# funcwj/setk

Measured on AMD Instinct MI355X. Metric: real-time-factor (audio-sec/wall-sec), 8-ch 16 kHz MVDR, higher is better.
Workload: dtype f32; 1 GPU; 8-ch 16 kHz oracle-mask MVDR, 30 s utterances, 125 per GPU (BASELINE configs[2] shard: 1000 at 8 GPUs), STFT 512/256/hann/center, inputs resident in HBM; utts_per_gpu=125, channels=8, frames=1876, beamformer=mvdr, parallelism=utterance-sharded x1

## Files before the change

setk_amd/build.py:

```python
import os
import subprocess
import sys
from concurrent.futures import ThreadPoolExecutor

HERE = os.path.dirname(os.path.abspath(__file__))
CSRC = os.path.join(HERE, "csrc")
OBJ = os.path.join(CSRC, "_obj")
LIB = os.path.join(HERE, "libsetk_hip.so")
SOURCES = ["pass1.hip", "pass1_mc.hip", "pass2.hip", "pass2_mc.hip", "solve.hip", "modular.hip", "cgmm.hip", "cgmm_bin.hip", "cgmm_k.hip", "wpe.hip", "auxiva.hip", "comm.hip", "hostio.hip",
           "capi_support.hip", "capi_handle.hip", "capi_stft.hip", "capi_modular.hip", "capi_fused.hip", "capi_cgmm.hip", "capi_wpe.hip", "capi_auxiva.hip"]
HEADERS = ["common.h", "fft512.h", "dpp.h", "covar_fold.h", "mcdft.h", "mcdft_tables.h", "capi.h", os.path.join("..", "..", "include", "setk_hip.h")]
ARCH = "gfx950"


def _hipcc():
    for cand in (os.environ.get("HIPCC"), "/opt/rocm/bin/hipcc", "hipcc"):
        if cand and (os.path.isabs(cand) and os.path.exists(cand) or not os.path.isabs(cand)):
            return cand
    return "hipcc"


def _stale(target, deps):
    if not os.path.exists(target):
        return True
    t = os.path.getmtime(target)
    return any(os.path.getmtime(d) > t for d in deps)


def build_library(force=False, verbose=False):
    os.makedirs(OBJ, exist_ok=True)
    import fcntl
    with open(os.path.join(OBJ, ".lock"), "w") as lock:
        fcntl.flock(lock, fcntl.LOCK_EX)
        return _build_locked(force, verbose)


def _build_locked(force, verbose):
    hdrs = [os.path.normpath(os.path.join(CSRC, h)) for h in HEADERS]
    flags = ["--offload-arch=" + ARCH, "-O3", "-std=c++17", "-fPIC", "-ffp-contract=fast",
             "-fno-slp-vectorize",
             "-Wno-unused-result"] + os.environ.get("SETK_HIPCC_FLAGS", "").split()
    extra = {"pass1.hip": ["-mllvm", "-amdgpu-sched-strategy=max-memory-clause"],
             "pass2_mc.hip": ["-mllvm", "-amdgpu-sched-strategy=max-ilp"],
             "pass2.hip": ["-mllvm", "-amdgpu-sched-strategy=max-ilp"],
             "solve.hip": ["-mllvm", "-amdgpu-sched-strategy=max-ilp"],
             "modular.hip": ["-mllvm", "-amdgpu-sched-strategy=max-ilp"],
             "cgmm.hip": ["-mllvm", "-amdgpu-sched-strategy=max-ilp"],
             "cgmm_bin.hip": ["-mllvm", "-amdgpu-sched-strategy=iterative-ilp"],
             "cgmm_k.hip": [],
             "wpe.hip": ["-mllvm", "-amdgpu-sched-strategy=max-ilp"],
             "auxiva.hip": [],
             "comm.hip": []}
    honor = {"solve.hip", "modular.hip"}
    jobs = []
    objs = []
    for src in SOURCES:
        s = os.path.join(CSRC, src)
        o = os.path.join(OBJ, src.replace(".hip", ".o"))
        objs.append(o)
        if force or _stale(o, [s] + hdrs):
            fl = [f if f != "-ffp-contract=fast" or src not in honor else "-ffp-contract=fast-honor-pragmas"
                  for f in flags]
            jobs.append([_hipcc()] + fl + extra.get(src, []) + ["-c", s, "-o", o])

    def run(cmd):
        if verbose:
            print(" ".join(cmd), file=sys.stderr)
        r = subprocess.run(cmd, capture_output=True, text=True)
        if r.returncode != 0:
            raise RuntimeError("hipcc failed:\n" + " ".join(cmd) + "\n" + r.stdout + r.stderr)
        return r

    if jobs:
        with ThreadPoolExecutor(max_workers=min(len(jobs), os.cpu_count() or 1)) as ex:
            list(ex.map(run, jobs))
    if force or jobs or _stale(LIB, objs):
        run([_hipcc(), "--offload-arch=" + ARCH, "-shared", "-fPIC", "-o", LIB] + objs)
    return LIB


if __name__ == "__main__":
    if "--units" in sys.argv:
        print(" ".join(s[:-len(".hip")] for s in SOURCES))
        sys.exit(0)
    print(build_library(force="--force" in sys.argv, verbose=True))
```

setk_amd/csrc/fft512.h:

```cpp
#pragma once
#include <hip/hip_runtime.h>

namespace setk {

typedef float2 cf;

#define SETK_DEV __device__ __forceinline__

#define SETK_GLOBAL __attribute__((address_space(1)))
typedef const SETK_GLOBAL float* gcfloat_p;
typedef float v2f __attribute__((ext_vector_type(2)));
typedef const SETK_GLOBAL v2f* gcfloat2_p;
template <class T>
SETK_DEV const SETK_GLOBAL T* gptr(const T* p) {
    return (const SETK_GLOBAL T*)p;
}

SETK_DEV cf cadd(cf a, cf b) { return make_float2(a.x + b.x, a.y + b.y); }
SETK_DEV cf csub(cf a, cf b) { return make_float2(a.x - b.x, a.y - b.y); }
SETK_DEV cf cmul(cf a, cf b) {
    return make_float2(a.x * b.x - a.y * b.y, a.x * b.y + a.y * b.x);
}
SETK_DEV cf cmulc(cf a, cf b) {
    return make_float2(a.x * b.x + a.y * b.y, a.y * b.x - a.x * b.y);
// ... 35 lines not shown
    v[4 * 1 + 1] = twid16<DIR, 1>(v[4 * 1 + 1]);
    v[4 * 2 + 1] = twid16<DIR, 2>(v[4 * 2 + 1]);
    v[4 * 3 + 1] = twid16<DIR, 3>(v[4 * 3 + 1]);
    v[4 * 1 + 2] = twid16<DIR, 2>(v[4 * 1 + 2]);
    v[4 * 2 + 2] = twid16<DIR, 4>(v[4 * 2 + 2]);
    v[4 * 3 + 2] = twid16<DIR, 6>(v[4 * 3 + 2]);
    v[4 * 1 + 3] = twid16<DIR, 3>(v[4 * 1 + 3]);
    v[4 * 2 + 3] = twid16<DIR, 6>(v[4 * 2 + 3]);
    v[4 * 3 + 3] = twid16<DIR, 9>(v[4 * 3 + 3]);
#pragma unroll
    for (int c = 0; c < 4; ++c)
        dft4<DIR>(v[4 * c], v[4 * c + 1], v[4 * c + 2], v[4 * c + 3]);
}

constexpr int kRow5 = 10;
__host__ __device__ constexpr int slot_entries(int row) { return 16 * row; }
__host__ __device__ constexpr int table_entries(int row) {
    return (row % 2 == 0) ? 2 * 16 * row + 16 * kRow5 : 640;
}
template <int ROW> struct LaneTab {
    static constexpr bool rows = (ROW % 2 == 0);
    static constexpr int estride = rows ? 1 : 16;
    static constexpr int lstride = rows ? ROW : 1;
    static constexpr int lstride5 = rows ? kRow5 : 1;
    static constexpr int size = rows ? 16 * ROW : 256;
};

template <int N, bool WIDE = true>
SETK_DEV void lds_row(const cf* row, cf (&out)[N]) {
    if (WIDE) {
        const float4* r4 = reinterpret_cast<const float4*>(__builtin_assume_aligned(row, 16));
#pragma unroll
        for (int n = 0; n < N / 2; ++n) {
            const float4 t = r4[n];
            out[2 * n] = make_float2(t.x, t.y);
            out[2 * n + 1] = make_float2(t.z, t.w);
        }
    } else {
#pragma unroll
        for (int n = 0; n < N; ++n) out[n] = row[n];
    }
}

template <int ROW>
SETK_DEV void fill_lane_tables(cf* win_l, cf* tw_l, cf* tw5_l, const float* window,
                               const float2* tw256, const float2* tw512, int tid, int nthreads) {
    for (int i = tid; i < 256; i += nthreads) {
        const int la = i & 15, j = i >> 4, n = la + 16 * j;
        typedef LaneTab<ROW> L;
        win_l[la * L::lstride + j * L::estride] = make_float2(window[2 * n], window[2 * n + 1]);
        tw_l[la * L::lstride + j * L::estride] = tw256[j * 16 + la];
    }
    for (int i = tid; i < 128; i += nthreads) {
        const int la = i & 15, m = i >> 4;
        tw5_l[la * LaneTab<ROW>::lstride5 + m * LaneTab<ROW>::estride] = tw512[la + 16 * m];
    }
}

template <int ROW>
SETK_DEV void apply_window(cf (&v)[16], const cf* win_row) {
    if (LaneTab<ROW>::rows) {
        const float4* w4 = reinterpret_cast<const float4*>(__builtin_assume_aligned(win_row, 16));
#pragma unroll
        for (int j = 0; j < 16; j += 2) {
            const float4 w = w4[j / 2];
            v[j] = make_float2(v[j].x * w.x, v[j].y * w.y);
            v[j + 1] = make_float2(v[j + 1].x * w.z, v[j + 1].y * w.w);
        }
    } else {
#pragma unroll
        for (int j = 0; j < 16; ++j) {
            const cf w = win_row[j * 16];
            v[j] = make_float2(v[j].x * w.x, v[j].y * w.y);
        }
    }
}

template <int DIR, int ROW, bool WIDE = (ROW % 2 == 0)>
SETK_DEV void fft256_stage_a_pad(cf (&v)[16], cf* slot, const cf* tw_row, int la) {
    dft16<DIR>(v);
    cf* dst = slot + la;
    if (WIDE) {
        const float4* w4 = reinterpret_cast<const float4*>(__builtin_assume_aligned(tw_row, 16));
#pragma unroll
        for (int q = 0; q < 16; q += 2) {
            const float4 w = w4[q / 2];
            cf t0 = v[dft16_pos(q)], t1 = v[dft16_pos(q + 1)];
            if (q) t0 = cmul(t0, make_float2(w.x, DIR > 0 ? -w.y : w.y));
            t1 = cmul(t1, make_float2(w.z, DIR > 0 ? -w.w : w.w));
            dst[q * ROW] = t0;
            dst[(q + 1) * ROW] = t1;
        }
    } else {
        cf wq[16];
        wq[1] = tw_row[16];
        wq[2] = tw_row[32];
#pragma unroll
        for (int q = 0; q < 16; ++q) {
            if (q + 3 < 16) wq[q + 3] = tw_row[(q + 3) * 16];
            cf t = v[dft16_pos(q)];
            if (q) {
                cf w = wq[q];
                if (DIR > 0) w.y = -w.y;
                t = cmul(t, w);
            }
            dst[q * ROW] = t;
        }
    }
}

template <int DIR, int ROW, bool WIDE = (ROW % 2 == 0)>
SETK_DEV void fft256_stage_b_pad(cf (&v)[16], const cf* slot, int la) {
    lds_row<16, WIDE>(slot + la * ROW, v);
    dft16<DIR>(v);
}

SETK_DEV void rfft_split(cf Zk, cf Zm, cf w, cf& Xk, cf& Xm) {
    cf A = make_float2(Zk.x + Zm.x, Zk.y - Zm.y);
    cf O = make_float2(Zk.y + Zm.y, Zm.x - Zk.x);
    cf B = cmul(w, O);
    Xk = cadd(A, B);
    Xm = make_float2(A.x - B.x, -(A.y - B.y));
}

SETK_DEV void irfft_merge(cf Yk, cf Ym, cf w, cf& Zk, cf& Zm) {
    cf E = make_float2(Yk.x + Ym.x, Yk.y - Ym.y);
    cf D = make_float2(Yk.x - Ym.x, Yk.y + Ym.y);
    cf O = cmulc(D, w);
    Zk = make_float2(E.x - O.y, E.y + O.x);
    Zm = make_float2(E.x + O.y, -E.y + O.x);
}

constexpr int kFrame = 512;

SETK_DEV int reflect_index(int i, int n) {
    if (i < 0) i = -i;
    if (i >= n) i = 2 * (n - 1) - i;
    return i;
}

template <class FloatPtr> struct RawPair;
template <> struct RawPair<gcfloat_p> {
    typedef gcfloat2_p ptr;
    static SETK_DEV cf get(ptr p, int i) {
        const v2f d = p[i];
        return make_float2(d.x, d.y);
    }
};
template <> struct RawPair<const float*> {
    typedef const float2* ptr;
    static SETK_DEV cf get(ptr p, int i) { return p[i]; }
};

template <class FloatPtr>
SETK_DEV void load_raw(cf (&v)[16], FloatPtr x, int n_samp, int s, int la, bool valid) {
    if (!valid) {
#pragma unroll
        for (int j = 0; j < 16; ++j) v[j] = make_float2(0.f, 0.f);
        return;
    }
    const bool interior = (s >= 0) && (s + kFrame <= n_samp) && ((((uintptr_t)(x + s)) & 7) == 0);
    if (interior) {
        typename RawPair<FloatPtr>::ptr p = (typename RawPair<FloatPtr>::ptr)(x + s);
#pragma unroll
        for (int j = 0; j < 16; ++j) v[j] = RawPair<FloatPtr>::get(p, la + 16 * j);
    } else {
#pragma unroll
        for (int j = 0; j < 16; ++j) {
            const int n = la + 16 * j;
            v[j] = make_float2(x[reflect_index(s + 2 * n, n_samp)],
                               x[reflect_index(s + 2 * n + 1, n_samp)]);
        }
    }
}

typedef const SETK_GLOBAL short* gcshort_p;
typedef const SETK_GLOBAL int* gcint_p;
SETK_DEV void load_raw_pcm(int (&v)[16], gcshort_p x, int n_samp, int s, int la, bool valid) {
    if (!valid) {
#pragma unroll
        for (int j = 0; j < 16; ++j) v[j] = 0;
        return;
    }
    const bool interior = (s >= 0) && (s + kFrame <= n_samp) && ((((uintptr_t)(x + s)) & 3) == 0);
    if (interior) {
        gcint_p p = (gcint_p)(x + s);
#pragma unroll
        for (int j = 0; j < 16; ++j) v[j] = p[la + 16 * j];
    } else {
#pragma unroll
        for (int j = 0; j < 16; ++j) {
            const int n = la + 16 * j;
            const int lo = x[reflect_index(s + 2 * n, n_samp)];
            const int hi = x[reflect_index(s + 2 * n + 1, n_samp)];
            v[j] = (lo & 0xffff) | (hi << 16);
        }
    }
}
SETK_DEV cf unpack_pcm(int v) { return make_float2((float)(short)(v & 0xffff), (float)(v >> 16)); }

SETK_DEV float qr_partner(float x) {
    int v = __builtin_bit_cast(int, x);
    v = __builtin_amdgcn_update_dpp(0, v, 0x140, 0xf, 0xf, true);
    v = __builtin_amdgcn_update_dpp(0, v, 0x121, 0xf, 0xf, true);
    return __builtin_bit_cast(float, v);
}

template <int ROW, bool WIDE = (ROW % 2 == 0)>
SETK_DEV void qr_stage23(cf* slot, float* nyq, const cf* tw5_row, int la) {
    cf v[16];
    fft256_stage_b_pad<-1, ROW, WIDE>(v, slot, la);
    const bool lane0 = (la == 0);
    cf* lo = slot + la;
    cf* mir = slot + (256 - 16 * 7) - la;
    cf t5[8];
    if (WIDE) {
        lds_row<8, true>(tw5_row, t5);
    } else {
        t5[0] = tw5_row[0];
        t5[1] = tw5_row[16];
    }
#pragma unroll
    for (int m = 0; m < 8; ++m) {
        if (!WIDE && m + 2 < 8) t5[m + 2] = tw5_row[16 * (m + 2)];
        const cf Zk = v[dft16_pos(m)];
        const cf src = v[dft16_pos(15 - m)];
        cf Zm = make_float2(qr_partner(src.x), qr_partner(src.y));
        const cf own = v[dft16_pos((16 - m) & 15)];
        Zm.x = lane0 ? own.x : Zm.x;
        Zm.y = lane0 ? own.y : Zm.y;
        cf Xk, Xm;
        rfft_split(Zk, Zm, t5[m], Xk, Xm);
        if (m == 0) {
            const cf Z128 = v[dft16_pos(8)];
            if (lane0) {
                slot[0] = make_float2(Xk.x, 0.f);
                *nyq = Xm.x;
                slot[128] = make_float2(2.f * Z128.x, -2.f * Z128.y);
            } else {
                lo[16 * m] = Xk;
                mir[16 * (7 - m)] = Xm;
            }
        } else {
            lo[16 * m] = Xk;
            mir[16 * (7 - m)] = Xm;
        }
    }
}

}
```

setk_amd/csrc/pass1.hip:

```cpp
#include "common.h"
#include "fft512.h"
#include "covar_fold.h"
#include <cstdio>
#include <type_traits>
#include <cstdlib>

namespace setk {

template <int C, bool DUMP, bool PCM = false>
__global__ __launch_bounds__(1024, 4) void stft_covar_kernel(Pass1Args a) {
    constexpr int NT = 1024;
    constexpr int TB = pass1_tile_frames(C);
    constexpr int NF = TB * C;
    constexpr int NP = npairs(C);
    constexpr int ND = PairSplit<C>::ND, NO = PairSplit<C>::NO;
    constexpr int NS = 32 / NF;
    constexpr int F = kBins, FP = kBinsPad;
    constexpr int ROW = 17;
    constexpr int SL = slot_entries(ROW);

    extern __shared__ __attribute__((aligned(16))) char smem[];
    cf* xt0 = reinterpret_cast<cf*>(smem);
    cf* win_l = xt0 + 2 * NF * SL;
    cf* tw_l = win_l + LaneTab<ROW>::size;
// ... 110 lines not shown
                for (int j = i; j < C; ++j) {
                    if (cnt == e) { ny_i = i; ny_j = j; }
                    ++cnt;
                }
        }
        float cur_s[TB], cur_n[TB], nxt_s[TB], nxt_n[TB];
        auto fetch_masks = [&](int tb_tile, float (&ms)[TB], float (&mn)[TB]) {
#pragma unroll
            for (int tt = 0; tt < TB; ++tt) {
                const int t = tb_tile + tt;
                float vs = 0.f, vn = 0.f;
                if (t < wi.t1) {
                    vs = gptr(ud.mask_s)[(size_t)t * F + f];
                    if (has_mn) vn = gptr(ud.mask_n)[(size_t)t * F + f];
                }
                ms[tt] = vs;
                mn[tt] = vn;
            }
        };
        if (!DUMP) fetch_masks(wi.t0, cur_s, cur_n);
        wg_barrier();
        wg_barrier();
        int buf = 0;
#pragma unroll 1
        for (int tb = wi.t0; tb < wi.t1; tb += TB, buf ^= 1) {
            const cf* xt = xt0 + buf * NF * SL;
            const float* xn = xn0 + buf * 32;
            if (DUMP) {
                for (int i = q; i < NF; i += 2) {
                    const int tt = i / C, c = i - tt * C;
                    const int t = tb + tt;
                    if (t < wi.t1) {
                        float2* base = a.spec_dump ? reinterpret_cast<float2*>(a.spec_dump)
                                                   : reinterpret_cast<float2*>(ud.wave_out);
                        float2* dst = base + ((size_t)c * T + t) * (a.dump_pitch ? a.dump_pitch : F);
                        dst[f] = xt[i * SL + f];
                        if (f == 0) dst[256] = make_float2(xn[i], 0.f);
                    }
                }
            } else {
                if (tb + TB < wi.t1) fetch_masks(tb + TB, nxt_s, nxt_n);
#pragma unroll
                for (int tt = 0; tt < TB; ++tt) {
                    cf x[C];
#pragma unroll
                    for (int c = 0; c < C; ++c) x[c] = xt[(tt * C + c) * SL + f];
                    const bool fvalid = tb + tt < wi.t1;
                    const float ws = clamp ? fminf(cur_s[tt], 1.f) : cur_s[tt];
                    const float wn = fvalid ? (has_mn ? cur_n[tt] : 1.f - ws) : 0.f;
                    if (q == 0) {
                        aux0 += ws;
                        aux1 += wn;
                        accumulate_half<C, 0>(x, ws, wn, dg_s, dg_n, of_s, of_n);
                    } else {
                        accumulate_half<C, 1>(x, ws, wn, dg_s, dg_n, of_s, of_n);
                    }
                    if (ny_active) {
                        const float prod_ny =
                            (ny_item < 2 * NP) ? xn[tt * C + ny_i] * xn[tt * C + ny_j] : 1.f;
                        const bool speech = (ny_item < NP) || (ny_item == 2 * NP);
                        const float w256 = nym[(buf * 2 + (speech ? 0 : 1)) * 8 + tt];
                        aux0 = fmaf(w256, prod_ny, aux0);
                    }
                }
#pragma unroll
                for (int tt = 0; tt < TB; ++tt) {
                    cur_s[tt] = nxt_s[tt];
                    cur_n[tt] = nxt_n[tt];
                }
            }
            wg_barrier();
        }
    }

    if (!DUMP) {
        if (wi.last) {
            const int covered = (T - 1) * a.g.hop - a.g.pad + kNfft;
            for (int c = 0; c < C; ++c)
                for (int i = covered + tid; i < n_samp; i += NT) {
                    if constexpr (PCM)
                        mx = fmaxf(mx, fabsf((float)((gcshort_p)gptr(ud.audio))[(size_t)c * ud.ch_stride + i]));
                    else
                        mx = fmaxf(mx, fabsf(gptr(ud.audio)[(size_t)c * n_samp + i]));
                }
        }
        if constexpr (PCM) mx *= 3.0517578125e-05f;
#pragma unroll
        for (int o = 32; o > 0; o >>= 1) mx = fmaxf(mx, __shfl_xor(mx, o));
        if ((tid & 63) == 0) red[tid >> 6] = mx;
        __syncthreads();
        if (tid == 0) {
            float bm = red[0];
#pragma unroll
            for (int w = 1; w < NT / 64; ++w) bm = fmaxf(bm, red[w]);
            atomicMax(a.norm_bits + wi.utt, __float_as_uint(bm));
        }
        if (wave >= 8) {
            float* P = a.partials + (size_t)wi.part * nplanes_partial(C) * FP;
            if (q == 0) {
                store_half<C, 0>(P, f, dg_s, dg_n, of_s, of_n);
                P[(4 * NP + 0) * FP + f] = aux0;
                P[(4 * NP + 1) * FP + f] = aux1;
            } else {
                store_half<C, 1>(P, f, dg_s, dg_n, of_s, of_n);
            }
            if (ny_active) {
                if (ny_item < NP) {
                    P[(0 * NP + ny_item) * FP + 256] = aux0;
                    P[(1 * NP + ny_item) * FP + 256] = 0.f;
                } else if (ny_item < 2 * NP) {
                    P[(2 * NP + ny_item - NP) * FP + 256] = aux0;
                    P[(3 * NP + ny_item - NP) * FP + 256] = 0.f;
                } else {
                    P[(4 * NP + ny_item - 2 * NP) * FP + 256] = aux0;
                }
            }
        }
    }
}

constexpr int kBmFrames = 64;
constexpr int kBmSlot = slot_entries(17) + 1;

__global__ __launch_bounds__(1024, 4) void stft_binmajor_kernel(Pass1Args a, int C) {
    constexpr int ROW = 17;
    constexpr int NT = 1024;
    extern __shared__ __attribute__((aligned(16))) char smem[];
    cf* xt = reinterpret_cast<cf*>(smem);
    cf* win_l = xt + kBmFrames * kBmSlot;
    cf* tw_l = win_l + LaneTab<ROW>::size;
    cf* tw5_l = tw_l + LaneTab<ROW>::size;
    float* xn = reinterpret_cast<float*>(win_l + table_entries(ROW));

    const int tid = threadIdx.x;
    const int wave = tid >> 6, lane = tid & 63;
    const int la = tid & 15, grp = tid >> 4;
    const WorkItem wi = a.items[blockIdx.x];
    const UttDesc ud = a.utts[wi.utt];
    const int n_samp = ud.num_samples, T = ud.num_frames;
    const int Tp = (T + 3) & ~3;
    cf* out = reinterpret_cast<cf*>(ud.wave_out);
    fill_lane_tables<ROW>(win_l, tw_l, tw5_l, a.window, a.tw256, a.tw512, tid, NT);
    const cf* win_row = win_l + la * LaneTab<ROW>::lstride;
    const cf* tw_row = tw_l + la * LaneTab<ROW>::lstride;
    const cf* tw5_row = tw5_l + la * LaneTab<ROW>::lstride5;
    cf* slot = xt + grp * kBmSlot;
    const int t = wi.t0 + grp;
    const bool valid = t < wi.t1;

    const int s0 = t * a.g.hop - a.g.pad;
    __syncthreads();
    for (int c = 0; c < C; ++c) {
        cf v[16];
        load_raw(v, gptr(ud.audio) + (size_t)c * n_samp, n_samp, s0, la, valid);
        apply_window<ROW>(v, win_row);
        fft256_stage_a_pad<-1, ROW>(v, slot, tw_row, la);
        __builtin_amdgcn_wave_barrier();
        qr_stage23<ROW>(slot, xn + grp, tw5_row, la);
        __syncthreads();
        {
            const int fr = 2 * (lane & 31), half = lane >> 5;
            const int t2 = wi.t0 + fr;
            for (int f = 2 * wave + half; f < kBins; f += 2 * (NT / 64)) {
                cf v0, v1;
                if (f < 256) {
                    v0 = xt[fr * kBmSlot + f];
                    v1 = xt[(fr + 1) * kBmSlot + f];
                } else {
                    v0 = make_float2(xn[fr], 0.f);
                    v1 = make_float2(xn[fr + 1], 0.f);
                }
                cf* dst = out + ((size_t)f * C + c) * Tp + t2;
                if (t2 + 1 < wi.t1)
                    *reinterpret_cast<float4*>(dst) = make_float4(v0.x, v0.y, v1.x, v1.y);
                else if (t2 < wi.t1)
                    *dst = v0;
            }
        }
        __syncthreads();
    }
}

hipError_t launch_stft_binmajor(int C, const Pass1Args& a, int n_items, hipStream_t s) {
    const size_t lds = (size_t)kBmFrames * kBmSlot * sizeof(cf) + table_entries(17) * sizeof(cf) +
                       kBmFrames * sizeof(float);
    hipError_t e = hipFuncSetAttribute(reinterpret_cast<const void*>(stft_binmajor_kernel),
                                       hipFuncAttributeMaxDynamicSharedMemorySize, (int)lds);
    if (e != hipSuccess) return e;
    hipLaunchKernelGGL(stft_binmajor_kernel, dim3(n_items), dim3(1024), lds, s, a, C);
    return hipGetLastError();
}

template <int C, bool DUMP, bool PCM = false>
static hipError_t launch_pass1_t(const Pass1Args& a, int n_items, hipStream_t s) {
    constexpr int NF = pass1_tile_frames(C) * C;
    const size_t lds = (size_t)2 * NF * slot_entries(17) * sizeof(cf) + table_entries(17) * sizeof(cf) +
                       (64 + 32 + 16) * sizeof(float);
    auto k = stft_covar_kernel<C, DUMP, PCM>;
    hipError_t e = hipFuncSetAttribute(reinterpret_cast<const void*>(k),
                                       hipFuncAttributeMaxDynamicSharedMemorySize, (int)lds);
    if (e != hipSuccess) return e;
    hipLaunchKernelGGL(k, dim3(n_items), dim3(1024), lds, s, a);
    return hipGetLastError();
}

hipError_t launch_pass1(int C, bool dump, const Pass1Args& a, int n_items, hipStream_t s, bool pcm16) {
    if (pcm16 && dump) return hipErrorInvalidValue;
#define SETK_CASE(c)                                                \
    case c:                                                         \
        if (dump) return launch_pass1_t<c, true>(a, n_items, s);     \
        if (pcm16) return launch_pass1_t<c, false, true>(a, n_items, s); \
        return launch_pass1_t<c, false>(a, n_items, s);
    switch (C) {
        SETK_CASE(1)
        SETK_CASE(2)
        SETK_CASE(3)
        SETK_CASE(4)
        SETK_CASE(5)
        SETK_CASE(6)
        SETK_CASE(7)
        SETK_CASE(8)
    }
#undef SETK_CASE
    return hipErrorInvalidValue;
}

__global__ __launch_bounds__(320) void covar_finalize_kernel(FinalizeArgs a) {
    const int f = threadIdx.x;
    const int u = blockIdx.z;
    const int C = a.num_channels;
    const int NP = npairs(C);
    const int planes_in = 4 * NP + 2;
    const int planes_out = a.with_ry ? 6 * NP : 4 * NP;
    const int e = blockIdx.y;
    if (f >= kBinsPad) return;
    const UttDesc ud = a.utts[u];
    float* out = a.covar + ((size_t)u * planes_out + e) * kBinsPad;
    if (f >= kBins) {
        out[f] = 0.f;
        return;
    }
    const float* P = a.partials + (size_t)ud.part0 * planes_in * kBinsPad;
    const size_t slab = (size_t)planes_in * kBinsPad;
    if (e < 4 * NP) {
        const int sel = e / (2 * NP);
        float acc = 0.f, den = 0.f;
        for (int p = 0; p < ud.nparts; ++p) {
            acc += P[p * slab + (size_t)e * kBinsPad + f];
            den += P[p * slab + (size_t)(4 * NP + sel) * kBinsPad + f];
        }
        const float sc = a.num_scale / fmaxf(den, 1e-6f);
        out[f] = acc * sc;
    } else {
        const int r = e - 4 * NP;
        float acc = 0.f;
        for (int p = 0; p < ud.nparts; ++p)
            acc += P[p * slab + (size_t)r * kBinsPad + f] +
                   P[p * slab + (size_t)(2 * NP + r) * kBinsPad + f];
        const float sc = a.num_scale / fmaxf((float)ud.num_frames, 1e-6f);
        out[f] = acc * sc;
    }
}

hipError_t launch_finalize(const FinalizeArgs& a, int n_utts, hipStream_t s) {
    const int NP = npairs(a.num_channels);
    const int planes_out = a.with_ry ? 6 * NP : 4 * NP;
    dim3 grid(1, planes_out, n_utts);
    hipLaunchKernelGGL(covar_finalize_kernel, grid, dim3(320), 0, s, a);
    return hipGetLastError();
}

}
```

setk_amd/csrc/pass2_mc.hip:

```cpp
#include "common.h"
#include "fft512.h"
#include "mcdft.h"
#include <cstdio>
#include <cstdlib>
#include <type_traits>

namespace setk {

constexpr int kP2McWavesPerSimd = 4;
constexpr int kP2McGroup = 2;
constexpr int p2mc_threads(bool pcm) { return pcm ? 1024 : 512; }

constexpr int kP2McTiles = 25;
size_t pass2_mc_lds_bytes(int C, bool pcm) {
    const size_t nw = p2mc_threads(pcm) / 64;
    const size_t wt = ((size_t)C * kBins * sizeof(cf) + 15) & ~(size_t)15;
    return wt + kP2McTiles * 1024 + 2048 + nw * kP2McGroup * 8 * mc::kOddPitch * sizeof(float) +
           nw * kP2McGroup * 16 * sizeof(float) + 64 + (pcm ? nw * C * 64 * sizeof(uint2) : 0);
}

SETK_DEV float row8_sum(float x) {
    int v = __builtin_bit_cast(int, x);
    x += __builtin_bit_cast(float, __builtin_amdgcn_update_dpp(0, v, 0xB1, 0xf, 0xf, true));
    v = __builtin_bit_cast(int, x);
    x += __builtin_bit_cast(float, __builtin_amdgcn_update_dpp(0, v, 0x4E, 0xf, 0xf, true));
    v = __builtin_bit_cast(int, x);
    x += __builtin_bit_cast(float, __builtin_amdgcn_update_dpp(0, v, 0x141, 0xf, 0xf, true));
    return x;
}
SETK_DEV float wave_max_nonneg(float x) {
    int v = __builtin_bit_cast(int, x);
    x = fmaxf(x, __builtin_bit_cast(float, __builtin_amdgcn_update_dpp(0, v, 0xB1, 0xf, 0xf, true)));
    v = __builtin_bit_cast(int, x);
    x = fmaxf(x, __builtin_bit_cast(float, __builtin_amdgcn_update_dpp(0, v, 0x4E, 0xf, 0xf, true)));
    v = __builtin_bit_cast(int, x);
    x = fmaxf(x, __builtin_bit_cast(float, __builtin_amdgcn_update_dpp(0, v, 0x141, 0xf, 0xf, true)));
    v = __builtin_bit_cast(int, x);
    x = fmaxf(x, __builtin_bit_cast(float, __builtin_amdgcn_update_dpp(0, v, 0x140, 0xf, 0xf, true)));
    const unsigned b = __builtin_bit_cast(unsigned, x);
    unsigned m = __builtin_amdgcn_readlane(b, 0);
    const unsigned m1 = __builtin_amdgcn_readlane(b, 16), m2 = __builtin_amdgcn_readlane(b, 32),
                   m3 = __builtin_amdgcn_readlane(b, 48);
    m = m > m1 ? m : m1;
    m = m > m2 ? m : m2;
    m = m > m3 ? m : m3;
    return __builtin_bit_cast(float, m);
}

template <int C, bool PCM = false>
__global__ __launch_bounds__(p2mc_threads(PCM), kP2McWavesPerSimd) void beamform_istft_mc_kernel(Pass2Args a) {
    constexpr int NT = p2mc_threads(PCM);
    constexpr int NW = NT / 64;
    constexpr int F = kBins;

    extern __shared__ __attribute__((aligned(16))) char smem[];
    char* p = smem;
    cf* wtab = reinterpret_cast<cf*>(p);
    p += ((size_t)C * F * sizeof(cf) + 15) & ~(size_t)15;
    mc::u4* tiles = reinterpret_cast<mc::u4*>(p);
    p += kP2McTiles * 1024;
    mc::f4* synr = reinterpret_cast<mc::f4*>(p);
    p += 2048;
    float* a16s = reinterpret_cast<float*>(p);
    p += (size_t)NW * kP2McGroup * 8 * mc::kOddPitch * sizeof(float);
    float* yodd_s = reinterpret_cast<float*>(p);
    p += NW * kP2McGroup * 16 * sizeof(float);
    float* red = reinterpret_cast<float*>(p);
    p += 64;
    uint2* carry_s = reinterpret_cast<uint2*>(p);

    const int tid = threadIdx.x;
    const int lane = tid & 63;
    const int wave = __builtin_amdgcn_readfirstlane(tid >> 6);
    const int c16 = lane & 15, g = lane >> 4;
    const WorkItem wi = a.items[blockIdx.x];
    const UttDesc ud = a.utts[wi.utt];
    const int n_samp = ud.num_samples;
    const int T = ud.num_frames;
    const int hop = kNfft / 2;
    const bool post_mask = (a.flags & 0x4) != 0;
    const bool clamp = (a.flags & 0x2) != 0;

    float in_sc = PCM ? 3.0517578125e-05f : 1.f, out_sc = 1.f;
    if (a.norm_bits) {
        const unsigned nb = a.norm_bits[wi.utt];
        int e = (int)((nb >> 23) & 0xff) - 126;
        e = (__builtin_bit_cast(float, nb) <= 1.f) ? 0 : (e > 100 ? 100 : e);
        in_sc *= __builtin_bit_cast(float, (unsigned)(127 - e) << 23);
        out_sc = __builtin_bit_cast(float, (unsigned)(127 + e) << 23);
    }
    {
        const cf* wsrc = reinterpret_cast<const cf*>(a.weight) + (size_t)wi.utt * C * kBinsPad;
        for (int i = tid; i < C * F; i += NT) {
            const int c = i / F, f = i - c * F;
            wtab[i] = wsrc[c * kBinsPad + f];
        }
    }
    mc::stage_tiles(tiles, a.mc_tab, mc::kW_BR_H, 10, tid, NT);
    mc::stage_tiles(tiles + 10 * 64, a.mc_tab, mc::kW_OT_H, 2, tid, NT);
    mc::stage_tiles(tiles + 12 * 64, a.mc_tab, mc::kW_MC_H, 8, tid, NT);
    for (int i = tid; i < 128; i += NT) {
        const int l = i & 63, t4 = i >> 6;
        const mc::f4 w = {a.mc_win[(4 * t4 + 0) * 64 + l] * in_sc, a.mc_win[(4 * t4 + 1) * 64 + l] * in_sc,
                          a.mc_win[(4 * t4 + 2) * 64 + l] * in_sc, a.mc_win[(4 * t4 + 3) * 64 + l] * in_sc};
        tiles[20 * 64 + i] = __builtin_bit_cast(mc::u4, w);
    }
    mc::stage_tiles(tiles + 22 * 64, a.mc_tab, mc::kW_TR, 3, tid, NT);
    for (int i = tid; i < 128; i += NT) {
        const int l = i & 63, hf = i >> 6;
        synr[i] = (mc::f4){a.mc_syn[(4 * hf + 0) * 64 + l] * out_sc, a.mc_syn[(4 * hf + 1) * 64 + l] * out_sc,
                           a.mc_syn[(4 * hf + 2) * 64 + l] * out_sc, a.mc_syn[(4 * hf + 3) * 64 + l] * out_sc};
    }
    struct { float tr[4], ti[4]; } K;
    float* yoddw = yodd_s + wave * kP2McGroup * 16;
    const int lane_bin = mc::bin_of(c16, g, 0);
    const cf* wl = wtab + lane_bin;
    const int lane_n = 64 * g + c16;
    float omax = 0.f;
    __syncthreads();

    const int per = (wi.t1 - wi.t0 + NW - 1) / NW;
    const int ta = wi.t0 + wave * per;
    const int tb = min(ta + per, wi.t1);
    const int tw = ta > 0 ? ta - 1 : ta;

    constexpr int R = kP2McGroup;
    float* a16g = a16s + wave * R * 8 * mc::kOddPitch;
    float carry[4] = {0.f, 0.f, 0.f, 0.f};
    auto chan = [&](int c) {
        if constexpr (PCM) return (gcshort_p)gptr(ud.audio) + (size_t)c * ud.ch_stride;
        else return gptr(ud.audio) + (size_t)c * n_samp;
    };
    uint2* carry_l = carry_s + (size_t)wave * C * 64 + lane;
    auto load_pair = [&](float (&v)[12], int (&nr)[4], int t0, int c, auto edge) __attribute__((always_inline)) {
        const auto x = chan(c);
        const int o = 64 * g + c16;
        const int s0 = min(t0, T - 1) * hop - a.g.pad, s1 = min(t0 + 1, T - 1) * hop - a.g.pad + 256;
        if constexpr (PCM) {
            const uint2 pk = carry_l[64 * c];
            v[0] = (float)(short)(pk.x & 0xffff);
            v[1] = (float)((int)pk.x >> 16);
            v[2] = (float)(short)(pk.y & 0xffff);
            v[3] = (float)((int)pk.y >> 16);
            if (!decltype(edge)::value) {
#pragma unroll
                for (int e = 0; e < 4; ++e) {
                    v[4 + e] = x[s0 + o + 256 + 16 * e];
                    nr[e] = x[s1 + o + 16 * e];
                }
            } else {
#pragma unroll
                for (int e = 0; e < 4; ++e) {
                    v[4 + e] = x[reflect_index(s0 + o + 256 + 16 * e, n_samp)];
                    nr[e] = x[reflect_index(s1 + o + 16 * e, n_samp)];
                }
            }
        } else {
            if (!decltype(edge)::value) {
#pragma unroll
                for (int e = 0; e < 4; ++e) {
                    v[e] = __builtin_nontemporal_load(&x[s0 + o + 16 * e]);
                    v[4 + e] = __builtin_nontemporal_load(&x[s0 + o + 256 + 16 * e]);
                }
#pragma unroll
                for (int e = 0; e < 4; ++e) v[8 + e] = x[s1 + o + 16 * e];
            } else {
#pragma unroll
                for (int e = 0; e < 4; ++e) {
                    v[e] = x[reflect_index(s0 + o + 16 * e, n_samp)];
                    v[4 + e] = x[reflect_index(s0 + o + 256 + 16 * e, n_samp)];
                    v[8 + e] = x[reflect_index(s1 + o + 16 * e, n_samp)];
                }
            }
        }
    };
    mc::f4 yr[R], yi[R];
    static_assert(R == 2, "the paired transform and the LDS carry are written for groups of two frames");
    float nxt[12];
    int nraw[4];
    auto group = [&](int t0, auto edge) __attribute__((always_inline)) {
#pragma unroll
        for (int k = 0; k < R; ++k) {
            yr[k] = (mc::f4){0.f, 0.f, 0.f, 0.f};
            yi[k] = (mc::f4){0.f, 0.f, 0.f, 0.f};
        }
#pragma unroll 1
        for (int c = 0; c < C; ++c) {
            float x0[8], x1[8];
#pragma unroll
            for (int e = 0; e < 4; ++e) {
                x0[e] = nxt[e];
                x0[4 + e] = nxt[4 + e];
                x1[e] = nxt[4 + e];
                if constexpr (PCM) x1[4 + e] = (float)nraw[e];
                else x1[4 + e] = nxt[8 + e];
            }
            if constexpr (PCM) {
                carry_l[64 * c] = make_uint2(__builtin_amdgcn_perm((unsigned)nraw[1], (unsigned)nraw[0], 0x05040100u),
                                             __builtin_amdgcn_perm((unsigned)nraw[3], (unsigned)nraw[2], 0x05040100u));
            }
            if (c + 1 < C) load_pair(nxt, nraw, t0, c + 1, edge);
            mc::f4 zr0, zi0, a16_0, zr1, zi1, a16_1;
            {
                asm volatile("" ::: "memory");
                const mc::f4 w0 = __builtin_bit_cast(mc::f4, tiles[20 * 64 + lane]);
                const mc::f4 w1 = __builtin_bit_cast(mc::f4, tiles[21 * 64 + lane]);
                const float win[8] = {w0[0], w0[1], w0[2], w0[3], w1[0], w1[1], w1[2], w1[3]};
                mc::forward2_t(x0, x1, win, [&](int i) { return mc::lds_h8(tiles, 12 + i, lane); },
                               [&](int i) { return __builtin_bit_cast(mc::f4, tiles[(22 + i) * 64 + lane]); },
                               zr0, zi0, a16_0, zr1, zi1, a16_1);
            }
            __builtin_amdgcn_sched_barrier(0);
            asm volatile("" ::: "memory");
            const cf* wc = wl + c * F;
            cf w[4];
#pragma unroll
            for (int r = 0; r < 4; ++r) w[r] = wc[32 * r];
            mc::store_a16(a16g, c, lane, a16_0);
            mc::store_a16(a16g + 8 * mc::kOddPitch, c, lane, a16_1);
#pragma unroll
            for (int r = 0; r < 4; ++r) {
                yr[0][r] = fmaf(zr0[r], w[r].x, fmaf(zi0[r], w[r].y, yr[0][r]));
                yi[0][r] = fmaf(zi0[r], w[r].x, fmaf(-zr0[r], w[r].y, yi[0][r]));
                yr[1][r] = fmaf(zr1[r], w[r].x, fmaf(zi1[r], w[r].y, yr[1][r]));
                yi[1][r] = fmaf(zi1[r], w[r].x, fmaf(-zr1[r], w[r].y, yi[1][r]));
            }
            __builtin_amdgcn_sched_barrier(0);
        }
    };
    auto span_is_edge = [&](int t0) {
        const int lo = t0 * hop - a.g.pad, hi = (t0 + R - 1) * hop - a.g.pad + kNfft;
        return lo < 0 || hi > n_samp || t0 + R > T;
    };
    auto request_group = [&](int t0) __attribute__((always_inline)) {
        if (span_is_edge(t0)) load_pair(nxt, nraw, t0, 0, std::true_type());
        else load_pair(nxt, nraw, t0, 0, std::false_type());
    };
    if constexpr (PCM) {
        if (tw < tb) {
#pragma unroll 1
            for (int c = 0; c < C; ++c) {
                const auto x = chan(c);
                const int s0 = tw * hop - a.g.pad, o = 64 * g + c16;
                int r[4];
#pragma unroll
                for (int e = 0; e < 4; ++e) r[e] = x[reflect_index(s0 + o + 16 * e, n_samp)];
                carry_l[64 * c] = make_uint2(__builtin_amdgcn_perm((unsigned)r[1], (unsigned)r[0], 0x05040100u),
                                             __builtin_amdgcn_perm((unsigned)r[3], (unsigned)r[2], 0x05040100u));
            }
        }
    }
    if (tw < tb) request_group(tw);
#pragma unroll 1
    for (int t0 = tw; t0 < tb; t0 += R) {
        const int nf = min(R, tb - t0);
        if (span_is_edge(t0)) group(t0, std::true_type());
        else group(t0, std::false_type());
        if (t0 + R < tb) request_group(t0 + R);
        const int t1 = min(t0 + 1, T - 1);
        int lt = lane;
        asm volatile("" : "+v"(lt));
        const int kf = (lt >> 3) & 1, co = lt & 7, c16 = lt & 15, g = lt >> 4;
        const bool odd_on = co < C;
        const cf* wo = wtab + (odd_on ? co : 0) * F + 16 + 64 * g;
        const int orow = 8 * kf + (odd_on ? co : C - 1);
        float yo[4];
        {
            asm volatile("" ::: "memory");
            const mc::f4 d = mc::odd_tile_row(a16g, mc::lds_h8(tiles, 10, lane), mc::lds_h8(tiles, 11, lane), lane, orow);
            const cf w0 = wo[0], w1 = wo[32];
            yo[0] = odd_on ? fmaf(d[0], w0.x, d[1] * w0.y) : 0.f;
            yo[1] = odd_on ? fmaf(d[1], w0.x, -d[0] * w0.y) : 0.f;
            yo[2] = odd_on ? fmaf(d[2], w1.x, d[3] * w1.y) : 0.f;
            yo[3] = odd_on ? fmaf(d[3], w1.x, -d[2] * w1.y) : 0.f;
#pragma unroll
            for (int i = 0; i < 4; ++i) yo[i] = row8_sum(yo[i]);
        }
        mc::f4 fr[R], fi[R];
#pragma unroll
        for (int k = 0; k < R; ++k) {
            fr[k] = yr[k];
            fi[k] = yi[k];
        }
        if (post_mask) {
            const float* mrow = ud.mask_s + (size_t)t0 * F;
            const unsigned dm = (unsigned)(t1 - t0) * F;
            unsigned mo = (unsigned)lane_bin, mq = 16u + 64u * (unsigned)g + (kf ? dm : 0u);
            asm volatile("" : "+v"(mo), "+v"(mq));
#pragma unroll
            for (int k = 0; k < R; ++k) {
#pragma unroll
                for (int r = 0; r < 4; ++r) {
                    float m = mrow[mo + (k ? dm : 0u) + 32 * r];
                    if (clamp) m = fminf(m, 1.f);
                    fr[k][r] *= m;
                    fi[k][r] *= m;
                }
            }
            float m0 = mrow[mq], m1 = mrow[mq + 32];
            if (clamp) { m0 = fminf(m0, 1.f); m1 = fminf(m1, 1.f); }
            yo[0] *= m0;
            yo[1] *= m0;
            yo[2] *= m1;
            yo[3] *= m1;
        }
        const float yom = fmaxf(fmaxf(fabsf(yo[0]), fabsf(yo[1])), fmaxf(fabsf(yo[2]), fabsf(yo[3])));
        float sc[R], isc[R];
#pragma unroll
        for (int k = 0; k < R; ++k) {
            fi[k][0] = (lane == 0) ? 0.f : fi[k][0];
            fi[k][3] = (lane == 32) ? 0.f : fi[k][3];
            float mxl = (kf == k) ? yom : 0.f;
#pragma unroll
            for (int r = 0; r < 4; ++r) mxl = fmaxf(mxl, fmaxf(fabsf(fr[k][r]), fabsf(fi[k][r])));
            const float mxw = wave_max_nonneg(mxl);
            int ex = (int)((__builtin_bit_cast(unsigned, mxw) >> 23) & 0xff);
            ex = ex < 16 ? 16 : (ex > 250 ? 250 : ex);
            sc[k] = __builtin_bit_cast(float, (unsigned)(264 - ex) << 23);
            isc[k] = __builtin_bit_cast(float, (unsigned)(ex - 10) << 23);
        }
        {
            const float scl = kf ? sc[1] : sc[0];
            if ((c16 & 7) == 0) *reinterpret_cast<mc::f4*>(yoddw + 16 * kf + 4 * g) = (mc::f4){yo[0] * scl, yo[1] * scl, yo[2] * scl, yo[3] * scl};
        }
        float e16[R];
        {
            float v[8];
            const mc::f4 v0 = *reinterpret_cast<const mc::f4*>(yoddw + 16 * (c16 & 1) + 8 * (g & 1));
            const mc::f4 v1 = *reinterpret_cast<const mc::f4*>(yoddw + 16 * (c16 & 1) + 8 * (g & 1) + 4);
            const float rowsel = c16 < R ? 1.f : 0.f;
#pragma unroll
            for (int e = 0; e < 4; ++e) {
                v[e] = v0[e] * rowsel;
                v[4 + e] = v1[e] * rowsel;
            }
            const mc::f4 d = mc::inv_odd_tile(v, mc::lds_h8(tiles, 8, lane), mc::lds_h8(tiles, 9, lane), lane);
            e16[0] = d[0];
            e16[1] = d[1];
        }
#pragma unroll
        for (int k = 0; k < R; ++k) {
#pragma unroll
            for (int r = 0; r < 4; ++r) {
                fr[k][r] *= sc[k];
                fi[k][r] *= sc[k];
            }
        }
        float bmid0[8], bmid1[8];
        {
            const mc::f4 tt0 = __builtin_bit_cast(mc::f4, tiles[22 * 64 + lane]);
            const mc::f4 tt1 = __builtin_bit_cast(mc::f4, tiles[23 * 64 + lane]);
#pragma unroll
            for (int r = 0; r < 4; ++r) {
                K.tr[r] = tt0[r];
                K.ti[r] = tt1[r];
            }
        }
        auto inv_tile = [&](int i) { return mc::lds_h8(tiles, i, lane); };
        mc::inverse2_a(fr[0], fi[0], e16[0], fr[1], fi[1], e16[1], inv_tile, K.tr, K.ti, bmid0, bmid1, lane);
        asm volatile("" ::: "memory");
        mc::f4 y0[R], y1[R];
        mc::inverse2_b(bmid0, bmid1, inv_tile, y0[0], y1[0], y0[1], y1[1]);
        const mc::f4 s0 = synr[lane], s1 = synr[64 + lane];
#pragma unroll
        for (int k = 0; k < R; ++k) {
            if (k >= nf) break;
            const int t = t0 + k;
            float blk[4];
#pragma unroll
            for (int r = 0; r < 4; ++r) blk[r] = fmaf(y0[k][r], s0[r] * isc[k], carry[r]);
            if (t == 0) {
#pragma unroll
                for (int r = 0; r < 4; ++r) blk[r] *= gptr(a.mc_edge)[r * 64 + lane];
            }
            if (t >= ta) {
                const int o = t * hop - a.g.pad + lane_n;
#pragma unroll
                for (int r = 0; r < 4; ++r) {
                    const int oo = o + 16 * r;
                    if (oo >= 0 && oo < ud.out_len) {
                        ud.wave_f32[oo] = blk[r];
                        omax = fmaxf(omax, fabsf(blk[r]));
                    }
                }
            }
#pragma unroll
            for (int r = 0; r < 4; ++r) carry[r] = y1[k][r] * (s1[r] * isc[k]);
        }
    }
// ... 60 lines not shown
```

Baseline: 2.138 million x real time (audio seconds per wall second, all GPUs).

## Double-buffer channel prefetch, wave-uniform interior loads, and scalar base addressing

In the multichannel pass-2 kernel, the per-channel body becomes a lambda, and for float input with five or more channels it ping-pongs between two prefetch buffers. This lets the next channel's load go into a separate register set rather than overwriting the one being consumed. Base addresses are forced into scalar registers so the loads use cheaper SGPR-based addressing. The raw-sample loaders now use a wave-wide ballot, so the fast interior path is taken uniformly across the wave, and the QR split stage selects its source before the DPP exchange. The build flags are also factored into a helper. The double buffers raise register pressure and may reduce occupancy.

```diff
diff --git a/setk_amd/build.py b/setk_amd/build.py
--- a/setk_amd/build.py
+++ b/setk_amd/build.py
@@ -35,9 +35,8 @@
         return _build_locked(force, verbose)
 
 
-def _build_locked(force, verbose):
-    hdrs = [os.path.normpath(os.path.join(CSRC, h)) for h in HEADERS]
-    flags = ["--offload-arch=" + ARCH, "-O3", "-std=c++17", "-fPIC", "-ffp-contract=fast",
+def unit_flags(src, arch=ARCH):
+    flags = ["--offload-arch=" + arch, "-O3", "-std=c++17", "-fPIC", "-ffp-contract=fast",
              "-fno-slp-vectorize",
              "-Wno-unused-result"] + os.environ.get("SETK_HIPCC_FLAGS", "").split()
     extra = {"pass1.hip": ["-mllvm", "-amdgpu-sched-strategy=max-memory-clause"],
@@ -52,6 +51,13 @@
              "auxiva.hip": [],
              "comm.hip": []}
     honor = {"solve.hip", "modular.hip"}
+    fl = [f if f != "-ffp-contract=fast" or src not in honor else "-ffp-contract=fast-honor-pragmas"
+          for f in flags]
+    return fl + extra.get(src, [])
+
+
+def _build_locked(force, verbose):
+    hdrs = [os.path.normpath(os.path.join(CSRC, h)) for h in HEADERS]
     jobs = []
     objs = []
     for src in SOURCES:
@@ -59,9 +65,7 @@
         o = os.path.join(OBJ, src.replace(".hip", ".o"))
         objs.append(o)
         if force or _stale(o, [s] + hdrs):
-            fl = [f if f != "-ffp-contract=fast" or src not in honor else "-ffp-contract=fast-honor-pragmas"
-                  for f in flags]
-            jobs.append([_hipcc()] + fl + extra.get(src, []) + ["-c", s, "-o", o])
+            jobs.append([_hipcc()] + unit_flags(src) + ["-c", s, "-o", o])
 
     def run(cmd):
         if verbose:
diff --git a/setk_amd/csrc/fft512.h b/setk_amd/csrc/fft512.h
--- a/setk_amd/csrc/fft512.h
+++ b/setk_amd/csrc/fft512.h
@@ -211,49 +211,54 @@
     static SETK_DEV cf get(ptr p, int i) { return p[i]; }
 };
 
-template <class FloatPtr>
+template <class FloatPtr, bool WAVE = true>
 SETK_DEV void load_raw(cf (&v)[16], FloatPtr x, int n_samp, int s, int la, bool valid) {
+    if (!WAVE && !valid) {
+#pragma unroll
+        for (int j = 0; j < 16; ++j) v[j] = make_float2(0.f, 0.f);
+        return;
+    }
+    const bool interior = valid && (s >= 0) && (s + kFrame <= n_samp) && ((((uintptr_t)(x + s)) & 7) == 0);
+    if (WAVE ? __builtin_expect(__builtin_amdgcn_ballot_w64(!interior) == 0, 1) : interior) {
+        typename RawPair<FloatPtr>::ptr p = (typename RawPair<FloatPtr>::ptr)(x + s);
+#pragma unroll
+        for (int j = 0; j < 16; ++j) v[j] = RawPair<FloatPtr>::get(p, la + 16 * j);
+        return;
+    }
     if (!valid) {
 #pragma unroll
         for (int j = 0; j < 16; ++j) v[j] = make_float2(0.f, 0.f);
         return;
     }
-    const bool interior = (s >= 0) && (s + kFrame <= n_samp) && ((((uintptr_t)(x + s)) & 7) == 0);
-    if (interior) {
-        typename RawPair<FloatPtr>::ptr p = (typename RawPair<FloatPtr>::ptr)(x + s);
-#pragma unroll
-        for (int j = 0; j < 16; ++j) v[j] = RawPair<FloatPtr>::get(p, la + 16 * j);
-    } else {
-#pragma unroll
-        for (int j = 0; j < 16; ++j) {
-            const int n = la + 16 * j;
-            v[j] = make_float2(x[reflect_index(s + 2 * n, n_samp)],
-                               x[reflect_index(s + 2 * n + 1, n_samp)]);
-        }
+#pragma unroll
+    for (int j = 0; j < 16; ++j) {
+        const int n = la + 16 * j;
+        v[j] = make_float2(x[reflect_index(s + 2 * n, n_samp)],
+                           x[reflect_index(s + 2 * n + 1, n_samp)]);
     }
 }
 
 typedef const SETK_GLOBAL short* gcshort_p;
 typedef const SETK_GLOBAL int* gcint_p;
 SETK_DEV void load_raw_pcm(int (&v)[16], gcshort_p x, int n_samp, int s, int la, bool valid) {
+    const bool interior = valid && (s >= 0) && (s + kFrame <= n_samp) && ((((uintptr_t)(x + s)) & 3) == 0);
+    if (__builtin_expect(__builtin_amdgcn_ballot_w64(!interior) == 0, 1)) {
+        gcint_p p = (gcint_p)(x + s);
+#pragma unroll
+        for (int j = 0; j < 16; ++j) v[j] = p[la + 16 * j];
+        return;
+    }
     if (!valid) {
 #pragma unroll
         for (int j = 0; j < 16; ++j) v[j] = 0;
         return;
     }
-    const bool interior = (s >= 0) && (s + kFrame <= n_samp) && ((((uintptr_t)(x + s)) & 3) == 0);
-    if (interior) {
-        gcint_p p = (gcint_p)(x + s);
-#pragma unroll
-        for (int j = 0; j < 16; ++j) v[j] = p[la + 16 * j];
-    } else {
-#pragma unroll
-        for (int j = 0; j < 16; ++j) {
-            const int n = la + 16 * j;
-            const int lo = x[reflect_index(s + 2 * n, n_samp)];
-            const int hi = x[reflect_index(s + 2 * n + 1, n_samp)];
-            v[j] = (lo & 0xffff) | (hi << 16);
-        }
+#pragma unroll
+    for (int j = 0; j < 16; ++j) {
+        const int n = la + 16 * j;
+        const int lo = x[reflect_index(s + 2 * n, n_samp)];
+        const int hi = x[reflect_index(s + 2 * n + 1, n_samp)];
+        v[j] = (lo & 0xffff) | (hi << 16);
     }
 }
 SETK_DEV cf unpack_pcm(int v) { return make_float2((float)(short)(v & 0xffff), (float)(v >> 16)); }
@@ -265,7 +270,7 @@
     return __builtin_bit_cast(float, v);
 }
 
-template <int ROW, bool WIDE = (ROW % 2 == 0)>
+template <int ROW, bool WIDE = (ROW % 2 == 0), bool PICK_FIRST = true>
 SETK_DEV void qr_stage23(cf* slot, float* nyq, const cf* tw5_row, int la) {
     cf v[16];
     fft256_stage_b_pad<-1, ROW, WIDE>(v, slot, la);
@@ -283,11 +288,11 @@
     for (int m = 0; m < 8; ++m) {
         if (!WIDE && m + 2 < 8) t5[m + 2] = tw5_row[16 * (m + 2)];
         const cf Zk = v[dft16_pos(m)];
-        const cf src = v[dft16_pos(15 - m)];
+        const cf oth = v[dft16_pos(15 - m)];
+        const cf own = v[dft16_pos((16 - m) & 15)];
+        const cf src = PICK_FIRST ? make_float2(lane0 ? own.x : oth.x, lane0 ? own.y : oth.y) : oth;
         cf Zm = make_float2(qr_partner(src.x), qr_partner(src.y));
-        const cf own = v[dft16_pos((16 - m) & 15)];
-        Zm.x = lane0 ? own.x : Zm.x;
-        Zm.y = lane0 ? own.y : Zm.y;
+        if (!PICK_FIRST) Zm = make_float2(lane0 ? own.x : Zm.x, lane0 ? own.y : Zm.y);
         cf Xk, Xm;
         rfft_split(Zk, Zm, t5[m], Xk, Xm);
         if (m == 0) {
diff --git a/setk_amd/csrc/pass1.hip b/setk_amd/csrc/pass1.hip
--- a/setk_amd/csrc/pass1.hip
+++ b/setk_amd/csrc/pass1.hip
@@ -286,11 +286,11 @@
     __syncthreads();
     for (int c = 0; c < C; ++c) {
         cf v[16];
-        load_raw(v, gptr(ud.audio) + (size_t)c * n_samp, n_samp, s0, la, valid);
+        load_raw<decltype(gptr(ud.audio)), false>(v, gptr(ud.audio) + (size_t)c * n_samp, n_samp, s0, la, valid);
         apply_window<ROW>(v, win_row);
         fft256_stage_a_pad<-1, ROW>(v, slot, tw_row, la);
         __builtin_amdgcn_wave_barrier();
-        qr_stage23<ROW>(slot, xn + grp, tw5_row, la);
+        qr_stage23<ROW, (ROW % 2 == 0), false>(slot, xn + grp, tw5_row, la);
         __syncthreads();
         {
             const int fr = 2 * (lane & 31), half = lane >> 5;
diff --git a/setk_amd/csrc/pass2_mc.hip b/setk_amd/csrc/pass2_mc.hip
--- a/setk_amd/csrc/pass2_mc.hip
+++ b/setk_amd/csrc/pass2_mc.hip
@@ -136,6 +136,16 @@
         const auto x = chan(c);
         const int o = 64 * g + c16;
         const int s0 = min(t0, T - 1) * hop - a.g.pad, s1 = min(t0 + 1, T - 1) * hop - a.g.pad + 256;
+        auto base = [&](int s) __attribute__((always_inline)) {
+            auto xs = x + s;
+            if constexpr (C > 2) asm volatile("" : "+s"(xs));
+            return xs;
+        };
+        const auto xa = base(s0), xb = base(s1);
+        auto at = [&](decltype(xa) xs, int s, int k) __attribute__((always_inline)) {
+            if constexpr (C > 2) return xs + ((unsigned)o + (unsigned)k);
+            else return x + (s + o + k);
+        };
         if constexpr (PCM) {
             const uint2 pk = carry_l[64 * c];
             v[0] = (float)(short)(pk.x & 0xffff);
@@ -145,8 +155,8 @@
             if (!decltype(edge)::value) {
 #pragma unroll
                 for (int e = 0; e < 4; ++e) {
-                    v[4 + e] = x[s0 + o + 256 + 16 * e];
-                    nr[e] = x[s1 + o + 16 * e];
+                    v[4 + e] = *at(xa, s0, 256 + 16 * e);
+                    nr[e] = *at(xb, s1, 16 * e);
                 }
             } else {
 #pragma unroll
@@ -159,11 +169,11 @@
             if (!decltype(edge)::value) {
 #pragma unroll
                 for (int e = 0; e < 4; ++e) {
-                    v[e] = __builtin_nontemporal_load(&x[s0 + o + 16 * e]);
-                    v[4 + e] = __builtin_nontemporal_load(&x[s0 + o + 256 + 16 * e]);
-                }
-#pragma unroll
-                for (int e = 0; e < 4; ++e) v[8 + e] = x[s1 + o + 16 * e];
+                    v[e] = __builtin_nontemporal_load(at(xa, s0, 16 * e));
+                    v[4 + e] = __builtin_nontemporal_load(at(xa, s0, 256 + 16 * e));
+                }
+#pragma unroll
+                for (int e = 0; e < 4; ++e) v[8 + e] = *at(xb, s1, 16 * e);
             } else {
 #pragma unroll
                 for (int e = 0; e < 4; ++e) {
@@ -176,56 +186,81 @@
     };
     mc::f4 yr[R], yi[R];
     static_assert(R == 2, "the paired transform and the LDS carry are written for groups of two frames");
-    float nxt[12];
-    int nraw[4];
+    constexpr bool kTwoBuf = !PCM && C >= 5;
+    float buf_a[12], buf_b[12];
+    int nraw_a[4], nraw_b[4];
+    auto channel = [&](const float (&cur)[12], const int (&craw)[4], float (&nx)[12], int (&nxraw)[4], int t0,
+                       int c, bool more, auto edge) __attribute__((always_inline)) {
+        float x0[8], x1[8];
+#pragma unroll
+        for (int e = 0; e < 4; ++e) {
+            x0[e] = cur[e];
+            x0[4 + e] = cur[4 + e];
+            x1[e] = cur[4 + e];
+            if constexpr (PCM) x1[4 + e] = (float)craw[e];
+            else x1[4 + e] = cur[8 + e];
+        }
+        if constexpr (PCM) {
+            carry_l[64 * c] = make_uint2(__builtin_amdgcn_perm((unsigned)craw[1], (unsigned)craw[0], 0x05040100u),
+                                         __builtin_amdgcn_perm((unsigned)craw[3], (unsigned)craw[2], 0x05040100u));
+        }
+        if (more) load_pair(nx, nxraw, t0, c + 1, edge);
+        mc::f4 zr0, zi0, a16_0, zr1, zi1, a16_1;
+        {
+            asm volatile("" ::: "memory");
+            const mc::f4 w0 = __builtin_bit_cast(mc::f4, tiles[20 * 64 + lane]);
+            const mc::f4 w1 = __builtin_bit_cast(mc::f4, tiles[21 * 64 + lane]);
+            const float win[8] = {w0[0], w0[1], w0[2], w0[3], w1[0], w1[1], w1[2], w1[3]};
+            mc::forward2_t(x0, x1, win, [&](int i) { return mc::lds_h8(tiles, 12 + i, lane); },
+                           [&](int i) { return __builtin_bit_cast(mc::f4, tiles[(22 + i) * 64 + lane]); },
+                           zr0, zi0, a16_0, zr1, zi1, a16_1);
+        }
+        __builtin_amdgcn_sched_barrier(0);
+        asm volatile("" ::: "memory");
+        const cf* wc = wl + c * F;
+        cf w[4];
+#pragma unroll
+        for (int r = 0; r < 4; ++r) w[r] = wc[32 * r];
+        mc::store_a16(a16g, c, lane, a16_0);
+        mc::store_a16(a16g + 8 * mc::kOddPitch, c, lane, a16_1);
+#pragma unroll
+        for (int r = 0; r < 4; ++r) {
+            yr[0][r] = fmaf(zr0[r], w[r].x, fmaf(zi0[r], w[r].y, yr[0][r]));
+            yi[0][r] = fmaf(zi0[r], w[r].x, fmaf(-zr0[r], w[r].y, yi[0][r]));
+            yr[1][r] = fmaf(zr1[r], w[r].x, fmaf(zi1[r], w[r].y, yr[1][r]));
+            yi[1][r] = fmaf(zi1[r], w[r].x, fmaf(-zr1[r], w[r].y, yi[1][r]));
+        }
+        if constexpr (kTwoBuf) {
+#pragma unroll
+            for (int k = 0; k < R; ++k) {
+                asm volatile("" : "+v"(yr[k][0]), "+v"(yr[k][1]), "+v"(yr[k][2]), "+v"(yr[k][3]),
+                                  "+v"(yi[k][0]), "+v"(yi[k][1]), "+v"(yi[k][2]), "+v"(yi[k][3]));
+            }
+        }
+        __builtin_amdgcn_sched_barrier(0);
+    };
     auto group = [&](int t0, auto edge) __attribute__((always_inline)) {
 #pragma unroll
         for (int k = 0; k < R; ++k) {
             yr[k] = (mc::f4){0.f, 0.f, 0.f, 0.f};
             yi[k] = (mc::f4){0.f, 0.f, 0.f, 0.f};
         }
+        if constexpr (decltype(edge)::value || !kTwoBuf) {
 #pragma unroll 1
-        for (int c = 0; c < C; ++c) {
-            float x0[8], x1[8];
-#pragma unroll
-            for (int e = 0; e < 4; ++e) {
-                x0[e] = nxt[e];
-                x0[4 + e] = nxt[4 + e];
-                x1[e] = nxt[4 + e];
-                if constexpr (PCM) x1[4 + e] = (float)nraw[e];
-                else x1[4 + e] = nxt[8 + e];
-            }
-            if constexpr (PCM) {
-                carry_l[64 * c] = make_uint2(__builtin_amdgcn_perm((unsigned)nraw[1], (unsigned)nraw[0], 0x05040100u),
-                                             __builtin_amdgcn_perm((unsigned)nraw[3], (unsigned)nraw[2], 0x05040100u));
-            }
-            if (c + 1 < C) load_pair(nxt, nraw, t0, c + 1, edge);
-            mc::f4 zr0, zi0, a16_0, zr1, zi1, a16_1;
-            {
-                asm volatile("" ::: "memory");
-                const mc::f4 w0 = __builtin_bit_cast(mc::f4, tiles[20 * 64 + lane]);
-                const mc::f4 w1 = __builtin_bit_cast(mc::f4, tiles[21 * 64 + lane]);
-                const float win[8] = {w0[0], w0[1], w0[2], w0[3], w1[0], w1[1], w1[2], w1[3]};
-                mc::forward2_t(x0, x1, win, [&](int i) { return mc::lds_h8(tiles, 12 + i, lane); },
-                               [&](int i) { return __builtin_bit_cast(mc::f4, tiles[(22 + i) * 64 + lane]); },
-                               zr0, zi0, a16_0, zr1, zi1, a16_1);
-            }
-            __builtin_amdgcn_sched_barrier(0);
-            asm volatile("" ::: "memory");
-            const cf* wc = wl + c * F;
-            cf w[4];
-#pragma unroll
-            for (int r = 0; r < 4; ++r) w[r] = wc[32 * r];
-            mc::store_a16(a16g, c, lane, a16_0);
-            mc::store_a16(a16g + 8 * mc::kOddPitch, c, lane, a16_1);
-#pragma unroll
-            for (int r = 0; r < 4; ++r) {
-                yr[0][r] = fmaf(zr0[r], w[r].x, fmaf(zi0[r], w[r].y, yr[0][r]));
-                yi[0][r] = fmaf(zi0[r], w[r].x, fmaf(-zr0[r], w[r].y, yi[0][r]));
-                yr[1][r] = fmaf(zr1[r], w[r].x, fmaf(zi1[r], w[r].y, yr[1][r]));
-                yi[1][r] = fmaf(zi1[r], w[r].x, fmaf(-zr1[r], w[r].y, yi[1][r]));
-            }
-            __builtin_amdgcn_sched_barrier(0);
+            for (int c = 0; c < C; ++c) channel(buf_a, nraw_a, buf_a, nraw_a, t0, c, c + 1 < C, edge);
+        } else {
+            int c = 0;
+#pragma unroll 1
+            for (; c + 2 < C; c += 2) {
+                channel(buf_a, nraw_a, buf_b, nraw_b, t0, c, true, edge);
+                channel(buf_b, nraw_b, buf_a, nraw_a, t0, c + 1, true, edge);
+            }
+            if constexpr (C % 2 == 0) {
+                channel(buf_a, nraw_a, buf_b, nraw_b, t0, c, true, edge);
+                channel(buf_b, nraw_b, buf_a, nraw_a, t0, c + 1, false, edge);
+            } else {
+                channel(buf_a, nraw_a, buf_b, nraw_b, t0, c, false, edge);
+            }
         }
     };
     auto span_is_edge = [&](int t0) {
@@ -233,8 +268,8 @@
         return lo < 0 || hi > n_samp || t0 + R > T;
     };
     auto request_group = [&](int t0) __attribute__((always_inline)) {
-        if (span_is_edge(t0)) load_pair(nxt, nraw, t0, 0, std::true_type());
-        else load_pair(nxt, nraw, t0, 0, std::false_type());
+        if (span_is_edge(t0)) load_pair(buf_a, nraw_a, t0, 0, std::true_type());
+        else load_pair(buf_a, nraw_a, t0, 0, std::false_type());
     };
     if constexpr (PCM) {
         if (tw < tb) {
```

Result: faster. 2.169 million x real time (audio seconds per wall second, all GPUs) (median of 6 runs) (+1.4%).
